# cyrillefavreau/Sol-R

Measured on AMD Instinct MI355X. Metric: Mrays/s @1920x1080, 3-bounce Cornell, higher is better.
Workload: dtype f32; 1 GPU; cornell 1920x1080, 3 bounces + shadow rays, 75 boxes / 29 primitives, one GPU, whole frame; rays_per_frame=6518779, closest_hit_walks_rank0=3506171, lane_nodes=206382796, lane_prim_tests=37557299, wave_nodes=3396811, wave_prim_tests=626627, wave_walks=106204, cost_ordered_launch_rank0=True, frames_in_flight=3, setup_frames_before_warmup=48, frames_delivered=9105, order_free_nodes=43, short_ray_lists=1, gather=none (one GPU), strips=equal rows, parallelism=tile1

## Files before the change

sol-r_amd/csrc/renderer.h:

```cpp
#ifndef SOLR_RENDERER_H
#define SOLR_RENDERER_H

#include <hip/hip_runtime.h>

#include "../../include/solr_hip.h"
#include "rt_device.h"

using namespace solrdev;

struct FrameArgs
{
    SceneInfo si;
    PostProcessingInfo ppi;
    float ox, oy, oz;
    float dx, dy, dz;
    float ax, ay, az, aw;
    Trig trig;
    float stepx, stepy;
    int firstRow;
    int nbRows;
    int tilesX;
    unsigned tileMagic;
    int tileShift;
    int fuseDefault;
// ... 46 lines not shown

struct PixelRecord
{
    float4 colorInfo;
    float4 sceneInfo;
};
static_assert(sizeof(PixelRecord) == sizeof(PostProcessingBuffer), "PixelRecord layout");


struct DepthHalo
{
    const float *above, *below;
    int nbAbove, nbBelow;
};

typedef void (*RendererFn)(const SceneArgs, const FrameArgs, PixelRecord *, int4 *, unsigned char *, unsigned long long *);
typedef void (*WalkBoundFn)(const SceneArgs, const char *, unsigned *, unsigned *);

namespace solrrows
{
struct Row
{
    int features;
    bool bothLoops;
};
constexpr Row ROWS[] = {
    {F_SPHERE | F_PLANE, true},
    {F_SPHERE | F_TRI, true},
    {F_SPHERE | F_CYL, true},
    {F_SPHERE | F_PLANE | F_TRI | F_CYL, false},
// ... 30 lines not shown
```

sol-r_amd/csrc/renderer_kernel.h:

```cpp
#ifndef SOLR_RENDERER_KERNEL_H
#define SOLR_RENDERER_KERNEL_H

#include "renderer.h"

using namespace solrdev;

template <int COUNT, int FEAT, bool VOLUME = false>
#ifndef SOLR_GENERIC_WAVES
#define SOLR_GENERIC_WAVES 0
#endif
#ifndef SOLR_WAVES_PER_EU
#define SOLR_WAVES_PER_EU 4
#endif
__global__ __launch_bounds__(WAVE, (SOLR_GENERIC_WAVES && (FEAT & F_TEX)) ? SOLR_GENERIC_WAVES : SOLR_WAVES_PER_EU) void k_standardRenderer(const SceneArgs SA, const FrameArgs F,
                                                           PixelRecord *__restrict__ pp,
                                                           int4 *__restrict__ ids, unsigned char *__restrict__ bitmap,
                                                           unsigned long long *__restrict__ counters)
{
    extern __shared__ float ldsStack[];
    const Scene S = makeScene(SA);
    const SceneInfo &si = F.si;
    const int lane = threadIdx.x;
    const unsigned entry = F.tileOrder ? F.tileOrder[blockIdx.x] : blockIdx.x;
    if (entry == ORDER_NOTHING)
        return;
    const int tile = (int)min(entry & ORDER_TILE_MASK, (unsigned)F.nbTiles - 1u);
    const int part = (int)((entry >> ORDER_PART_SHIFT) & 31u);
    unsigned long long clock0 = 0ull;
    if (F.tileClock || F.tileCost)
        clock0 = __builtin_amdgcn_s_memrealtime();
    const int ty = F.tileMagic ? (int)(__umulhi((unsigned)tile, F.tileMagic) >> F.tileShift) : tile;
    const int tx = tile - ty * F.tilesX;
    const int x = tx * TILE_W + (lane & (TILE_W - 1));
    const int yLocal = ty * TILE_H + (lane >> SOLR_TILE_W_LOG2);
    const int W = si.size.x;
    const bool mine = part == 0 || ((((lane & (TILE_W - 1)) >> (SOLR_TILE_W_LOG2 - SOLR_SPLIT_LOG2)) |
// ... 65 lines not shown
        rayD.y = rayD.y + F.stepy * (float)(yGlobal - (si.size.y / 2));
    }
    rayO = vectorRotation(rayO, rotationCenter, F.trig);
    rayD = vectorRotation(rayD, rotationCenter, F.trig);

    v3 color = V(0.f, 0.f, 0.f);
    if (!antialiasingActivated && (volume || si.pathTracingIteration >= NB_MAX_ITERATIONS))
    {
        const int k = si.pathTracingIteration % 4;
        rayD.x += (k == 0) ? 3.f : (k == 1) ? 5.f : (k == 2) ? -3.f : -5.f;
        rayD.y += (k == 0) ? 5.f : (k == 1) ? -3.f : (k == 2) ? -5.f : 3.f;
    }
    const bool anaglyph = (FEAT & F_FULL) && (si.cameraType == ctAnaglyph);
    const bool fishEye = (FEAT & F_FULL) && (si.cameraType == ctPanoramic);
    const bool vision = (FEAT & F_FULL) && (si.cameraType == ctVR);
    const bool plainStore = anaglyph || fishEye || vision;
    v3 leftEye = V(0.f, 0.f, 0.f);
    const int nbRays = antialiasingActivated ? 5 : (anaglyph ? 2 : 1);
#pragma unroll 1
    for (int I = 0; I < nbRays; ++I)
    {
        v3 rO = rayO;
        v3 rD = rayD;
        if (anaglyph)
        {
            const float stepx = F.stepx, stepy = F.stepy;
            rO = V((I == 0) ? F.ox - si.eyeSeparation : F.ox + si.eyeSeparation, F.oy, F.oz);
            rD = V(F.dx - stepx * (float)(x - (si.size.x / 2)), F.dy + stepy * (float)(yGlobal - (si.size.y / 2)), F.dz);
            rO = vectorRotation(rO, V(0.f, 0.f, 0.f), F.trig);
            rD = vectorRotation(rD, V(0.f, 0.f, 0.f), F.trig);
        }
        if (vision)
        {
            const float focus = fabsf(F.focusDepth - F.oz);
            const float eyeSeparation = si.eyeSeparation * (F.dz / focus);
            const int halfWidth = si.size.x / 2;
// ... 51 lines not shown
            }
            if (I >= 2)
            {
                rO.x += -3.f;
                rO.y += -5.f;
            }
            if (I >= 3)
            {
                rO.x += -5.f;
                rO.y += 3.f;
            }
        }
        v3 c;
        if constexpr (volume)
        {
            c = launchVolumeRendering<COUNT, FEAT>(S, active, gindex, rO, rD, si, F.ppi, id, cs, cnt);
            c = V(0.f + c.x, 0.f + c.y, 0.f + c.z);
        }
        else
            c = launchRayTracing<COUNT, FEAT>(S, active, gindex, rO, rD, si, dof, id, cs, cnt);
        if (anaglyph)
        {
            if (I == 0)
                leftEye = c;
            else
                color = V((leftEye.x * 0.299f + leftEye.y * 0.587f + leftEye.z * 0.114f) + 0.f, 0.f + c.y, 0.f + c.z);
        }
        else
            color = color + c;
    }

    SOLR_T(const unsigned long long tEpilogue0 = SOLR_NOW();)
    int tileAgain = tile, partAgain = part, laneAgain = (int)__builtin_amdgcn_mbcnt_hi(~0u, __builtin_amdgcn_mbcnt_lo(~0u, 0u));
    asm volatile("" : "+s"(tileAgain), "+s"(partAgain), "+v"(laneAgain));
    const int tyAgain = F.tileMagic ? (int)(__umulhi((unsigned)tileAgain, F.tileMagic) >> F.tileShift) : tileAgain;
    const int xAgain = (tileAgain - tyAgain * F.tilesX) * TILE_W + (laneAgain & (TILE_W - 1));
    const int yAgain = tyAgain * TILE_H + (laneAgain >> SOLR_TILE_W_LOG2);
    const int index = ((xAgain < si.size.x) && (yAgain < F.nbRows)) ? yAgain * si.size.x + xAgain : 0;
    const int gindexAgain = (F.firstRow + yAgain) * si.size.x + xAgain;

    if ((!plainStore || vision) && si.advancedIllumination == aiRandomIllumination)
    {
        int rindex = (gindexAgain + si.timestamp) % MAX_BITMAP_SIZE;
        float rv = rnd(S, rindex);
        color.x += si.backgroundColor.x * rv * 5.f;
        color.y += si.backgroundColor.y * rv * 5.f;
        color.z += si.backgroundColor.z * rv * 5.f;
    }
    if (antialiasingActivated)
    {
        color.x /= 5.f;
        color.y /= 5.f;
        color.z /= 5.f;
    }

    if (active)
    {
        float4 ppColor = make_float4(0.f, 0.f, 0.f, 0.f);
        float4 ppScene = make_float4(0.f, 0.f, 0.f, 0.f);
        if (si.pathTracingIteration > 0)
        {
            ppColor = pp[index].colorInfo;
            ppScene = pp[index].sceneInfo;
        }
        if (si.pathTracingIteration == 0)
            ppColor.w = dof;
        if (plainStore)
        {
            if (si.pathTracingIteration <= NB_MAX_ITERATIONS)
            {
                ppColor.x = color.x;
                ppColor.y = color.y;
                ppColor.z = color.z;
            }
            else
            {
                ppColor.x += color.x;
                ppColor.y += color.y;
                ppColor.z += color.z;
            }
        }
        else if (si.pathTracingIteration <= NB_MAX_ITERATIONS)
        {
            ppColor.x = color.x;
            ppColor.y = color.y;
            ppColor.z = color.z;
            ppScene.x = color.x;
            ppScene.y = color.y;
            ppScene.z = color.z;
        }
        else
        {
            ppScene.x = (id.z > 0) ? fmaxf(ppScene.x, color.x) : color.x;
            ppScene.y = (id.z > 0) ? fmaxf(ppScene.y, color.y) : color.y;
            ppScene.z = (id.z > 0) ? fmaxf(ppScene.z, color.z) : color.z;
            ppColor.x += ppScene.x;
            ppColor.y += ppScene.y;
            ppColor.z += ppScene.z;
        }
        pp[index].colorInfo = ppColor;
        pp[index].sceneInfo = ppScene;
        if ((FEAT & F_STREAM) && (F.fuseDefault & 4))
        {
            typedef int FourInts __attribute__((ext_vector_type(4)));
            const FourInts four = {id.x, id.y, id.z, id.w};
            asm volatile("global_store_dwordx4 %0, %1, off sc1" ::"v"(ids + index), "v"(four) : "memory");
        }
        else
            ids[index] = id;

        if (F.fuseDefault)
        {
            v3 c = V(ppColor.x, ppColor.y, ppColor.z);
            if (si.pathTracingIteration > NB_MAX_ITERATIONS)
            {
                float d = (float)(si.pathTracingIteration - NB_MAX_ITERATIONS + 1);
                c.x /= d;
                c.y /= d;
                c.z /= d;
            }
            if ((FEAT & F_STREAM) && (F.fuseDefault & 2))
                makeColor<true>(si, c, bitmap, index);
            else
                makeColor(si, c, bitmap, index);
        }
    }
    if ((FEAT & F_STREAM) && (F.fuseDefault & 2))
    {
        asm volatile("s_waitcnt vmcnt(0)" ::: "memory");
        const unsigned units = partAgain ? 1u : (unsigned)SPLIT_PARTS;
        unsigned before = 0u;
        if (laneAgain == 0)
            before = __hip_atomic_fetch_add(F.rowDone + 64 * tyAgain, units, __ATOMIC_RELAXED, __HIP_MEMORY_SCOPE_AGENT);
        before = (unsigned)__builtin_amdgcn_readfirstlane((int)before);
        if (before + units == F.streamSerial * (unsigned)(F.tilesX * SPLIT_PARTS) && laneAgain == 0)
        {
            const StreamPlan *plan = F.streamPlan;
            int band = 0;
            while (band + 1 < plan->bands && tyAgain >= plan->firstRow[band + 1])
                ++band;
            const int rows = plan->firstRow[band + 1] - plan->firstRow[band];
            const unsigned rowsBefore = __hip_atomic_fetch_add(plan->bandDone + 64 * band, 1u, __ATOMIC_RELAXED, __HIP_MEMORY_SCOPE_AGENT);
            if (rowsBefore + 1u == F.streamSerial * (unsigned)rows)
                __hip_atomic_store(plan->hostWord + band, F.streamSerial, __ATOMIC_RELAXED, __HIP_MEMORY_SCOPE_SYSTEM);
        }
    }

    if (F.tileClock && laneAgain == 0)
    {
        F.tileClock[2 * tileAgain] = clock0;
        F.tileClock[2 * tileAgain + 1] = __builtin_amdgcn_s_memrealtime();
    }
    if (F.tileCost && laneAgain == 0)
    {
        const unsigned cost = (unsigned)(__builtin_amdgcn_s_memrealtime() - clock0);
        F.tileCost[tileAgain] = partAgain ? (unsigned)(SOLR_SPLIT_LOG2 + 1) * cost : cost;
    }
#ifdef SOLR_TIMING
    if (COUNT == 0 && laneAgain == 0 && counters)
    {
        unsigned long long *slot = counters + 16 + 16ull * blockIdx.x;
        slot[0] += SOLR_NOW() - tKernel0;
        slot[8] += cnt.tShade;
        slot[9] += cnt.tTrace;
        slot[10] += SOLR_NOW() - tEpilogue0;
        slot[1] += cnt.tClosest;
        slot[2] += cnt.tShadow;
        slot[3] += cnt.tNode;
        slot[4] += cnt.tLeaf;
        slot[5] += (unsigned long long)cnt.nAdvance;
        slot[6] += (unsigned long long)cnt.nLeaf;
        slot[7] += 1ull;
        slot[11] += cnt.tClosestPrimary;
        slot[12] += cnt.tAgain;
        slot[13] += ((unsigned long long)cnt.nAgain << 32) | cnt.nAgainLanes;
        slot[14] += ((unsigned long long)cnt.nAdvanceFirst << 32) | cnt.nAdvanceAgain;
        slot[15] += (unsigned long long)cnt.nChecked;
    }
#endif
    if (COUNT == 2 && lane == 0)
        ((int4 *)cnt.record)[0] = make_int4((int)cnt.ordinal, 0, 0, 0);
    if (COUNT == 1)
    {
        unsigned int vals[4] = {cnt.closest, cnt.shadow, cnt.boxes, cnt.prims};
#pragma unroll
        for (int k = 0; k < 4; ++k)
        {
            unsigned int v = vals[k];
            for (int off = 32; off > 0; off >>= 1)
                v += __shfl_xor(v, off, 64);
            if (lane == 0)
                atomicAdd(&counters[k], (unsigned long long)v);
        }
        if (lane == 0)
        {
            atomicAdd(&counters[4], (unsigned long long)cnt.wNodes);
            atomicAdd(&counters[5], (unsigned long long)cnt.wPrims);
            atomicAdd(&counters[6], (unsigned long long)cnt.wClosest);
            atomicAdd(&counters[7], (unsigned long long)cnt.wShadow);
        }
    }
}

template <int FEAT>
__global__ __launch_bounds__(WAVE, SOLR_WAVES_PER_EU) void k_walkBound(const SceneArgs SA, const char *__restrict__ records,
                                                                       unsigned *__restrict__ visits, unsigned *__restrict__ skipped)
{
    extern __shared__ float ldsStack[];
    const Scene S = makeScene(SA);
    const int lane = threadIdx.x;
    const char *slot = records + (size_t)blockIdx.x * SOLR_WALK_SLOT_BYTES;
    const int4 *head = (const int4 *)slot;
    const float4 *rays = (const float4 *)(slot + 16 * (SOLR_WALK_SLOTS + 1));
    const int recorded = __builtin_amdgcn_readfirstlane(head[0].x);
// ... 64 lines not shown
```

sol-r_amd/csrc/rt_device.h:

```cpp
#pragma once

#include <hip/hip_runtime.h>
#include "pow_table.h"

#include "../../include/solr_types.h"
#include "scene_layout.h"

namespace solrdev
{
#define SOLR_DEV __device__ __forceinline__

struct v3
{
    float x, y, z;
};

SOLR_DEV v3 V(float x, float y, float z)
{
    v3 r;
    r.x = x;
    r.y = y;
    r.z = z;
    return r;
}
// ... 434 lines not shown


enum Feature
{
    F_SPHERE = 1,
    F_PROC = 2,
    F_CYL = 4,
    F_ELL = 8,
    F_TRI = 16,
    F_PLANE = 32,
    F_TEX = 64,
    F_FULL = 128,
    F_ALL = 255,
    F_DEEP = 256,
    F_STACK = 512,
    F_STREAM = 1024
};
#define SOLR_LDS_STACK_SLOTS 3

struct Hit
{
    v3 intersection;
    v3 normal;
    v3 areas;
    float shadowIntensity;
};

SOLR_DEV bool ellipsoidIntersection(const SceneInfo &si, v3 p0, v3 size, const WalkRay &ray, Hit &h)
{
    h.shadowIntensity = 1.f;
    v3 O_C = ray.o - p0;
    v3 dir = ray.dn;
// ... 816 lines not shown
}

SOLR_DEV bool longRay(v3 d)
{
    const float dd = dot(d, d);
    return dd >= 4.f && dd <= 1.0e24f;
}

SOLR_DEV bool tightRay(const WalkRay &r, const SceneInfo &si)
{
    return longRay(r.d) && r.d.x != 0.f && r.d.y != 0.f && r.d.z != 0.f && fabsf(r.o.x) <= si.viewDistance &&
           fabsf(r.o.y) <= si.viewDistance && fabsf(r.o.z) <= si.viewDistance;
}

template <int COUNT, int FEAT>
SOLR_DEV bool closestHitWalk(const Scene &S, const SceneInfo &si, bool active, v3 origin, v3 target, int iteration,
                             int currentMaterialId, int &closestPrimitive, v3 &closestIntersection,
                             v3 &closestNormal, v3 &closestAreas, v3 &colorBox, Counters &cnt)
{
    bool intersections = false;
    if (ballot(active) == 0ull)
        return false;
    SOLR_T(const unsigned long long tw0 = SOLR_NOW();)
    float minDistance = (iteration < 2) ? si.viewDistance : si.viewDistance / (iteration + 1);
    const WalkRay r = makeWalkRay(origin, target - origin);
    if (active)
        countAdd<COUNT>(cnt.closest, 1);
    countAdd<COUNT>(cnt.wClosest, 1);

    const bool fastBoxes = S.orderedBoxes && (ballot(active && !finiteRay(r)) == 0ull);
    const bool showBoxes = (FEAT & F_FULL) && si.renderBoxes != 0;
    const bool tidy = COUNT != 1 && fastBoxes && S.nested && !showBoxes;
    const bool freeOrder =
        tidy && S.nbBoxesFree > 0 && ballot(active && !longRay(r.d)) == 0ull;
    constexpr bool thinLeaves = (FEAT & F_PLANE) != 0;
    const bool tight = thinLeaves && tidy && S.tightLists && ballot(active && !tightRay(r, si)) == 0ull;
    const float ddShort = dot(r.d, r.d);
// ... 346 lines not shown
            break;
        SOLR_T(++cnt.nChecked;)
        const bool again = lanesNow && (intersections ? !(second > minDistance * rivalScale + slack) : bandHit);
        if (ballot(again) == 0ull)
            break;
        SOLR_T(++cnt.nAgain; cnt.nAgainLanes += (unsigned)__builtin_popcountll(ballot(again));)
        lanesNow = again;
        minDistance = again ? initialDistance : minDistance;
        intersections = again ? false : intersections;
    }
    SOLR_T(cnt.tClosest += SOLR_NOW() - tw0; if (iteration == 0) cnt.tClosestPrimary += SOLR_NOW() - tw0;)
    return intersections;
}

template <int COUNT, int FEAT>
SOLR_DEV float shadowWalk(const Scene &S, const SceneInfo &si, bool active, v3 lampCenter, v3 origin, int lightId,
                          int iteration, v3 &color, int objectId, Counters &cnt)
{
    float result = 0.f;
    color = V(0.f, 0.f, 0.f);
    if (ballot(active) == 0ull)
        return 0.f;
    SOLR_T(const unsigned long long tw0 = SOLR_NOW();)
    WalkRay r = makeWalkRay(origin, lampCenter - origin);
    r.o = origin + r.dn * si.rayEpsilon;
    const float minDistance = (iteration < 2) ? si.viewDistance : si.viewDistance / (iteration + 1);
    const float lengthOL = length(r.d);
    if (active)
        countAdd<COUNT>(cnt.shadow, 1);
    countAdd<COUNT>(cnt.wShadow, 1);

    const bool fastBoxes = S.orderedBoxes && (ballot(active && !finiteRay(r)) == 0ull);
    const bool tidy = COUNT != 1 && fastBoxes && S.nested;
    const bool freeOrder = tidy && S.nbBoxesFree > 0 && (S.opaqueShadows & SHADOWS_OPAQUE) &&
                           ballot(active && !(longRay(r.d) && minDistance >= 2.f)) == 0ull;
    const bool lampCut = tidy && !freeOrder && (S.opaqueShadows & SHADOWS_LAMP_CUTOFF);
    Scene W = S;
// ... 278 lines not shown
        }
    }
    else if (textured)
    {
        const float2 vt0 = make_float2(primRow(S, pi, ROW_N0).w, primRow(S, pi, ROW_N1).w);
        const float4 T = primRow(S, pi, ROW_UV);
        const float2 vt1 = make_float2(primRow(S, pi, ROW_N2).w, T.x);
        const float2 vt2 = make_float2(T.y, T.z);
        c = triangleUVMapping(si, vt0, vt1, vt2, mh.attributes.y, mh.color, loadMaterialCold(S, materialId), S.textures,
                              areas, o);
    }
    return c;
}

template <int COUNT, int FEAT>
SOLR_DEV v3 primitiveShader(const Scene &S, bool active, int index, const SceneInfo &si, v3 origin, v3 &normal,
                            int objectId, v3 intersection, v3 areas, v3 &closestColor, int iteration,
                            float &shadowIntensity, v3 &totalBlinn, float4 &attributes, Counters &cnt)
{
    SOLR_T(const unsigned long long tShade0 = SOLR_NOW();)
    const int pi = active ? objectId : 0;
    const int type = asint(primRow(S, pi, ROW_P0_TYPE).w) & PRIM_TYPE_MASK;
    const int materialId = asint(primRow(S, pi, ROW_SIZE_MAT).w);
    const int primIndex = asint(primRow(S, pi, ROW_P1_INDEX).w);
    const MaterialHot mh = loadMaterialHot(S, materialId);
    v3 lampsColor = V(0.f, 0.f, 0.f);
    v3 intersectionColor = V(0.f, 0.f, 0.f);
    float4 specular = make_float4(mh.specular.x, mh.specular.y, mh.specular.z, 0.f);
    float ambientOcclusion = 0.f;
    bool shade = active;

    if (active)
    {
        shadowIntensity = 0.f;
        v3 bumpNormal = V(0.f, 0.f, 0.f);
// ... 3 lines not shown
        normal = normal + bumpNormal;
        normal = normalize(normal);
        if (mh.attributes.z == 1)
            shade = false;
    }
    const bool wire = active && !shade;

    if (si.graphicsLevel > glNoShading)
    {
        if (shade)
        {
            closestColor.x *= mh.innerIllumination.x;
            closestColor.y *= mh.innerIllumination.x;
            closestColor.z *= mh.innerIllumination.x;
        }
        for (int cpt = 0; cpt < S.nbLights; ++cpt)
        {
            const int cptLamp =
                (si.pathTracingIteration >= NB_MAX_ITERATIONS) ? (si.pathTracingIteration % S.nbLights) : 0;
            const LightPlane li = loadLight(S, cptLamp);
            const int lightPrimitiveId = asint(li.location.w);
            const int lightMaterialId = li.materialId;
            const MaterialHot m = loadMaterialHot(S, lightMaterialId < 0 ? 0 : lightMaterialId);
            const bool lit = shade && (lightPrimitiveId != primIndex);

            v3 center = V4(li.location);
            const int t = (index + si.timestamp) % (MAX_BITMAP_SIZE - 3);
            if (si.pathTracingIteration >= NB_MAX_ITERATIONS)
            {
                float a = m.innerIllumination.y * 10.f * si.pathTracingIteration / si.maxPathTracingIterations;
                center.x += rnd(S, t) * a;
                center.y += rnd(S, t + 1) * a;
// ... 1 lines not shown
            }
            v3 lightRay = center - intersection;
            const float lightRayLength = length(lightRay);
            const bool inRange = lit && (lightRayLength < m.innerIllumination.z);
            v3 shadowColor = V(0.f, 0.f, 0.f);
            float lambert = 0.f;
            if (inRange)
            {
                lightRay = normalize(lightRay);
                lambert = mh.innerIllumination.x + dot(normal, lightRay);
            }
            const bool wantShadow = inRange && lambert > 0.f && si.graphicsLevel > 3 && iteration < 4 &&
                                    mh.innerIllumination.x == 0.f;
            {
                v3 sc;
                float s = shadowWalk<COUNT, FEAT>(S, si, wantShadow, center, intersection, lightPrimitiveId, iteration, sc,
                                            objectId, cnt);
                if (wantShadow)
                {
                    shadowIntensity = s;
                    shadowColor = sc;
                }
            }
            if (inRange)
            {
                float photonEnergy = sqrt_ieee(lightRayLength / m.innerIllumination.z);
                photonEnergy = (photonEnergy > 1.f) ? 1.f : photonEnergy;
                photonEnergy = (photonEnergy < 0.f) ? 0.f : photonEnergy;
                lambert *= (lambert < 0.f) ? -mh.transparency : 1.f;
                if (lightMaterialId != MATERIAL_NONE)
                    lambert *= m.innerIllumination.x;
                else
                    lambert *= li.color.w;
                if (mh.innerIllumination.w != 0.f)
                    lambert *= (1.f + rnd(S, t) * mh.innerIllumination.w * 100.f);
                lambert *= (1.f - shadowIntensity);
                lambert += si.backgroundColor.w;
                lambert *= (1.f - photonEnergy);
                lampsColor.x += lambert * li.color.x - shadowColor.x;
                lampsColor.y += lambert * li.color.y - shadowColor.y;
// ... 169 lines not shown
struct V3Ref
{
    float &x, &y, &z;
    SOLR_DEV V3Ref(const ColorStack &cs, int field) : x(cs.coldf(field)), y(cs.coldf(field + 1)), z(cs.coldf(field + 2)) {}
    SOLR_DEV operator v3() const { return V(x, y, z); }
    SOLR_DEV const V3Ref &operator=(const v3 &v) const
    {
        x = v.x;
        y = v.y;
        z = v.z;
        return *this;
    }
};

template <int COUNT, int FEAT>
SOLR_DEV v3 launchRayTracing(const Scene &S, bool active, int index, v3 rayO, v3 rayD, const SceneInfo &si,
                             float &depthOfField, int4 &primitiveXYId, const ColorStack &cs, Counters &cnt)
{
    SOLR_T(const unsigned long long tTrace0 = SOLR_NOW();)
    v3 intersectionColor = V(0.f, 0.f, 0.f);
    v3 closestIntersection = V(0.f, 0.f, 0.f);
    v3 normal = V(0.f, 0.f, 0.f);
    int closestPrimitive = -1;
    bool carryon = true;
    const V3Ref roO(cs, C_ROO), roD(cs, C_ROD);
    roO = rayO;
    roD = rayD;
    float &initialRefraction = cs.coldf(C_REFRACTION);
    initialRefraction = 1.f;
    int iteration = 0;
    int &lastIteration = cs.coldi(C_LASTIT);
    lastIteration = 0;
    int &idX = cs.coldi(C_ID_X), &idZ = cs.coldi(C_ID_Z), &idW = cs.coldi(C_ID_W);
    idX = -1;
// ... 42 lines not shown
    v3 ptO = V(0.f, 0.f, 0.f), ptD = V(0.f, 0.f, 0.f);
    float pathTracingRatio = 0.f;
    v3 pathTracingColor = V(0.f, 0.f, 0.f);
    bool useGlobalIllumination = false;
    bool test = true;

    v3 rBlinn = V(0.f, 0.f, 0.f);
    bool running = active;
    int phase = 0;

    while (true)
    {
        bool want;
        v3 tO, tD;
        int tIter, tMat;
        if (phase == 0)
        {
            running = running && (iteration < currentMaxIteration) && (rayLength < si.viewDistance) && carryon;
            if (ballot(running) == 0ull)
            {
                phase = 1;
                continue;
            }
            want = running;
            tO = roO;
            tD = roD;
            tIter = iteration;
            tMat = currentMaterialId;
        }
        else if (phase == 1)
// ... 2 lines not shown
            tO = rrO;
            tD = rrD;
            tIter = reflectedRays;
            tMat = currentMaterialId;
        }
        else
        {
            want = active && useGlobalIllumination && si.advancedIllumination == aiFull;
            tO = ptO;
            tD = ptD;
            tIter = 30;
            tMat = MATERIAL_NONE;
        }

        v3 areas = V(0.f, 0.f, 0.f);
        const bool hit = closestHitWalk<COUNT, FEAT>(S, si, want, tO, tD, tIter, tMat, closestPrimitive,
                                               closestIntersection, normal, areas, colorBox, cnt);
        const bool hitLane = want && hit;

        const int cp = hitLane ? closestPrimitive : 0;
        const int cpMaterial = asint(primRow(S, cp, ROW_SIZE_MAT).w);
        const MaterialHot cm = loadMaterialHot(S, cpMaterial < 0 ? 0 : cpMaterial);
        float4 attributes = make_float4(0.f, 0.f, 0.f, 0.f);
        bool shadeLane = hitLane;
        int shadeIteration = tIter;

        if (phase == 0)
        {
            if (running)
                carryon = hit;
            attributes = make_float4(cm.reflection, cm.transparency, cm.refraction, cm.opacity);
            if (hitLane)
            {
                currentMaterialId = cpMaterial;
                if (iteration == 0)
                {
                    cs.set(0, V(0.f, 0.f, 0.f));
                    cs.at(0, 3) = 1.f;
                    latestIntersection = closestIntersection;
                    dofCold = length(closestIntersection - tO);
                    if (giEnabled && cm.innerIllumination.x == 0.f)
                    {
                        int t = (index + si.pathTracingIteration * 100 + si.timestamp) % (MAX_BITMAP_SIZE - 3);
// ... 30 lines not shown
                        cs.at(0, 2) = cm.color.z * cm.innerIllumination.x * pathTracingRatio;
                        test = false;
                    }
                    else
                    {
                        cs.at(0, 0) = cm.color.x * pathTracingRatio;
                        cs.at(0, 1) = cm.color.y * pathTracingRatio;
                        cs.at(0, 2) = cm.color.z * pathTracingRatio;
                    }
                }
                if (test)
                {
                    pathTracingRatio *= STANDARD_LUNINANCE_STRENGTH;
                    if (cm.innerIllumination.x == 0.f)
                    {
                        cs.at(0, 0) -= si.shadowIntensity;
                        cs.at(0, 1) -= si.shadowIntensity;
                        cs.at(0, 2) -= si.shadowIntensity;
                    }
                    else
                        shadeLane = true;
                }
            }
            shadeIteration = lastIteration;
        }

        const v3 shaded = primitiveShader<COUNT, FEAT>(S, shadeLane, index, si, tO, normal, closestPrimitive,
                                                 closestIntersection, areas, closestColor, shadeIteration,
                                                 shadowIntensity, rBlinn, attributes, cnt);

        if (phase == 0)
        {
            if (hitLane)
            {
                v3 colorIt = shaded;
                float contribution;
                v3 reflectedTarget = V(0.f, 0.f, 0.f);
                idZ = (int)((float)idZ + cm.innerIllumination.x * 256);

                float segmentLength = length(closestIntersection - latestIntersection);
                latestIntersection = closestIntersection;

                float transparency = attributes.y;
                float a = 0.f;
                if (attributes.y != 0.f)
                {
                    float refraction = attributes.z;
// ... 84 lines not shown
        else if (phase == 1)
        {
            if (hitLane)
            {
                cs.template add<SP>(reflectedRays, V(shaded.x * reflectedRatio, shaded.y * reflectedRatio, shaded.z * reflectedRatio));
                idW = (int)(shadowIntensity * 255);
            }
            if (!giPass)
                break;
            phase = 2;
        }
        else
        {
            if (shadeLane)
                pathTracingColor = shaded;
            if (active && !hitLane && si.skyboxMaterialId != MATERIAL_NONE)
            {
                pathTracingColor = skyboxMapping<FEAT>(S, si, ptO, ptD);
                pathTracingRatio *= SKYBOX_LUNINANCE_STRENGTH;
            }
            if (active && test)
            {
                cs.at(0, 0) += pathTracingColor.x * pathTracingRatio;
                cs.at(0, 1) += pathTracingColor.y * pathTracingRatio;
                cs.at(0, 2) += pathTracingColor.z * pathTracingRatio;
            }
            break;
        }
    }

// ... 13 lines not shown
                const float4 cell = bs.template take<SP>(i);
                v3 ci = V(cell.x, cell.y, cell.z);
                float k = cell.w;
                next.x = ci.x * (1.f - k) + next.x * k;
                next.y = ci.y * (1.f - k) + next.y * k;
                next.z = ci.z * (1.f - k) + next.z * k;
            }
            intersectionColor = next;
            intersectionColor.x += recursiveBlinn.x;
            intersectionColor.y += recursiveBlinn.y;
            intersectionColor.z += recursiveBlinn.z;
        }
        else
            intersectionColor = cs.get(0);

        float D1 = si.viewDistance * 0.95f;
        const float dofNow = dofCold;
        if (si.atmosphericEffect == aeFog && dofNow > D1)
        {
            float D2 = si.viewDistance * 0.05f;
            float a = dofNow - D1;
            float b = 1.f - (a / D2);
            intersectionColor.x = intersectionColor.x * b + si.backgroundColor.x * (1.f - b);
            intersectionColor.y = intersectionColor.y * b + si.backgroundColor.y * (1.f - b);
            intersectionColor.z = intersectionColor.z * b + si.backgroundColor.z * (1.f - b);
        }
        intersectionColor.x -= colorBox.x;
        intersectionColor.y -= colorBox.y;
        intersectionColor.z -= colorBox.z;
    }
// ... 163 lines not shown
```

Baseline: 27680 Mrays/s.

## Read scene and frame args from kernarg segment to cut live registers

The renderer kernel now reads SceneArgs and FrameArgs through the kernarg segment pointer instead of copying them into locals. An opaque zero-offset helper (again<F_ARGS>) makes the compiler reload fields at each use rather than keep them live across the trace, shade and epilogue phases. The aim is lower SGPR/VGPR pressure and less spilling in the large kernel, at the cost of extra scalar loads. Triangle and textured variants keep their old behaviour.

```diff
diff --git a/sol-r_amd/csrc/renderer.h b/sol-r_amd/csrc/renderer.h
--- a/sol-r_amd/csrc/renderer.h
+++ b/sol-r_amd/csrc/renderer.h
@@ -84,6 +84,26 @@
     int nbAbove, nbBelow;
 };
 
+struct RendererArgs
+{
+    SceneArgs SA;
+    FrameArgs F;
+    PixelRecord *pp;
+    int4 *ids;
+    unsigned char *bitmap;
+    unsigned long long *counters;
+    __device__ __forceinline__ const Scene &scene() const { return *(const Scene *)&SA; }
+};
+static_assert(sizeof(Scene) == sizeof(SceneArgs) && alignof(Scene) == alignof(SceneArgs), "Scene is SceneArgs, retyped");
+static_assert(offsetof(Scene, offBoxes) == offsetof(SceneArgs, offBoxes) && offsetof(Scene, nbRandoms) == offsetof(SceneArgs, nbRandoms) &&
+                  offsetof(Scene, offLeaf) == offsetof(SceneArgs, offLeaf) && offsetof(Scene, sortedLists) == offsetof(SceneArgs, sortedLists),
+              "Scene is SceneArgs, retyped");
+static_assert(offsetof(RendererArgs, SA) == 0 && sizeof(RendererArgs) <= 512, "the kernel-argument segment of k_standardRenderer");
+__device__ __forceinline__ const RendererArgs &rendererArgs()
+{
+    return *(const RendererArgs *)(const SOLR_CONST_AS char *)__builtin_amdgcn_kernarg_segment_ptr();
+}
+
 typedef void (*RendererFn)(const SceneArgs, const FrameArgs, PixelRecord *, int4 *, unsigned char *, unsigned long long *);
 typedef void (*WalkBoundFn)(const SceneArgs, const char *, unsigned *, unsigned *);
 
diff --git a/sol-r_amd/csrc/renderer_kernel.h b/sol-r_amd/csrc/renderer_kernel.h
--- a/sol-r_amd/csrc/renderer_kernel.h
+++ b/sol-r_amd/csrc/renderer_kernel.h
@@ -12,14 +12,21 @@
 #ifndef SOLR_WAVES_PER_EU
 #define SOLR_WAVES_PER_EU 4
 #endif
-__global__ __launch_bounds__(WAVE, (SOLR_GENERIC_WAVES && (FEAT & F_TEX)) ? SOLR_GENERIC_WAVES : SOLR_WAVES_PER_EU) void k_standardRenderer(const SceneArgs SA, const FrameArgs F,
-                                                           PixelRecord *__restrict__ pp,
-                                                           int4 *__restrict__ ids, unsigned char *__restrict__ bitmap,
-                                                           unsigned long long *__restrict__ counters)
+__global__ __launch_bounds__(WAVE, (SOLR_GENERIC_WAVES && (FEAT & F_TEX)) ? SOLR_GENERIC_WAVES : SOLR_WAVES_PER_EU) void k_standardRenderer(const SceneArgs, const FrameArgs,
+                                                           PixelRecord *__restrict__,
+                                                           int4 *__restrict__, unsigned char *__restrict__,
+                                                           unsigned long long *__restrict__)
 {
     extern __shared__ float ldsStack[];
-    const Scene S = makeScene(SA);
+    constexpr int ARGS = FEAT | F_ARGS;
+    constexpr int TRACE = (FEAT & (F_TRI | F_TEX)) ? FEAT : ARGS;
+    const RendererArgs &A = rendererArgs();
+    const FrameArgs &F = A.F;
+    const Scene &S = A.scene();
     const SceneInfo &si = F.si;
+    PixelRecord *__restrict__ const pp = A.pp;
+    int4 *__restrict__ const ids = A.ids;
+    unsigned long long *__restrict__ const counters = A.counters;
     const int lane = threadIdx.x;
     const unsigned entry = F.tileOrder ? F.tileOrder[blockIdx.x] : blockIdx.x;
     if (entry == ORDER_NOTHING)
@@ -115,12 +122,13 @@
     const bool anaglyph = (FEAT & F_FULL) && (si.cameraType == ctAnaglyph);
     const bool fishEye = (FEAT & F_FULL) && (si.cameraType == ctPanoramic);
     const bool vision = (FEAT & F_FULL) && (si.cameraType == ctVR);
-    const bool plainStore = anaglyph || fishEye || vision;
     v3 leftEye = V(0.f, 0.f, 0.f);
     const int nbRays = antialiasingActivated ? 5 : (anaglyph ? 2 : 1);
 #pragma unroll 1
     for (int I = 0; I < nbRays; ++I)
     {
+        const FrameArgs &F = again<(FEAT & F_FULL) ? ARGS : 0>(A.F);
+        const SceneInfo &si = F.si;
         v3 rO = rayO;
         v3 rD = rayD;
         if (anaglyph)
@@ -202,11 +210,11 @@
         v3 c;
         if constexpr (volume)
         {
-            c = launchVolumeRendering<COUNT, FEAT>(S, active, gindex, rO, rD, si, F.ppi, id, cs, cnt);
+            c = launchVolumeRendering<COUNT, TRACE>(S, active, gindex, rO, rD, si, F.ppi, id, cs, cnt);
             c = V(0.f + c.x, 0.f + c.y, 0.f + c.z);
         }
         else
-            c = launchRayTracing<COUNT, FEAT>(S, active, gindex, rO, rD, si, dof, id, cs, cnt);
+            c = launchRayTracing<COUNT, TRACE>(S, active, gindex, rO, rD, si, dof, id, cs, cnt);
         if (anaglyph)
         {
             if (I == 0)
@@ -218,174 +226,187 @@
             color = color + c;
     }
 
-    SOLR_T(const unsigned long long tEpilogue0 = SOLR_NOW();)
-    int tileAgain = tile, partAgain = part, laneAgain = (int)__builtin_amdgcn_mbcnt_hi(~0u, __builtin_amdgcn_mbcnt_lo(~0u, 0u));
-    asm volatile("" : "+s"(tileAgain), "+s"(partAgain), "+v"(laneAgain));
-    const int tyAgain = F.tileMagic ? (int)(__umulhi((unsigned)tileAgain, F.tileMagic) >> F.tileShift) : tileAgain;
-    const int xAgain = (tileAgain - tyAgain * F.tilesX) * TILE_W + (laneAgain & (TILE_W - 1));
-    const int yAgain = tyAgain * TILE_H + (laneAgain >> SOLR_TILE_W_LOG2);
-    const int index = ((xAgain < si.size.x) && (yAgain < F.nbRows)) ? yAgain * si.size.x + xAgain : 0;
-    const int gindexAgain = (F.firstRow + yAgain) * si.size.x + xAgain;
-
-    if ((!plainStore || vision) && si.advancedIllumination == aiRandomIllumination)
-    {
-        int rindex = (gindexAgain + si.timestamp) % MAX_BITMAP_SIZE;
-        float rv = rnd(S, rindex);
-        color.x += si.backgroundColor.x * rv * 5.f;
-        color.y += si.backgroundColor.y * rv * 5.f;
-        color.z += si.backgroundColor.z * rv * 5.f;
-    }
-    if (antialiasingActivated)
-    {
-        color.x /= 5.f;
-        color.y /= 5.f;
-        color.z /= 5.f;
-    }
-
-    if (active)
-    {
-        float4 ppColor = make_float4(0.f, 0.f, 0.f, 0.f);
-        float4 ppScene = make_float4(0.f, 0.f, 0.f, 0.f);
-        if (si.pathTracingIteration > 0)
-        {
-            ppColor = pp[index].colorInfo;
-            ppScene = pp[index].sceneInfo;
-        }
-        if (si.pathTracingIteration == 0)
-            ppColor.w = dof;
-        if (plainStore)
-        {
-            if (si.pathTracingIteration <= NB_MAX_ITERATIONS)
+    {
+        SOLR_T(const unsigned long long tEpilogue0 = SOLR_NOW();)
+        int tileAgain = tile, partAgain = part, laneAgain = (int)__builtin_amdgcn_mbcnt_hi(~0u, __builtin_amdgcn_mbcnt_lo(~0u, 0u));
+        asm volatile("" : "+s"(tileAgain), "+s"(partAgain), "+v"(laneAgain));
+        const RendererArgs &E = again<ARGS>(A);
+        const FrameArgs &F = E.F;
+        const Scene &S = E.scene();
+        const SceneInfo &si = F.si;
+        PixelRecord *__restrict__ const pp = E.pp;
+        int4 *__restrict__ const ids = E.ids;
+        unsigned char *__restrict__ const bitmap = E.bitmap;
+        unsigned long long *__restrict__ const counters = E.counters;
+        const bool antialiasingActivated = (FEAT & F_FULL) && (si.cameraType == ctAntialiazed);
+        const bool vision = (FEAT & F_FULL) && (si.cameraType == ctVR);
+        const bool plainStore = vision || ((FEAT & F_FULL) && (si.cameraType == ctAnaglyph || si.cameraType == ctPanoramic));
+        const int tyAgain = F.tileMagic ? (int)(__umulhi((unsigned)tileAgain, F.tileMagic) >> F.tileShift) : tileAgain;
+        const int xAgain = (tileAgain - tyAgain * F.tilesX) * TILE_W + (laneAgain & (TILE_W - 1));
+        const int yAgain = tyAgain * TILE_H + (laneAgain >> SOLR_TILE_W_LOG2);
+        const int index = ((xAgain < si.size.x) && (yAgain < F.nbRows)) ? yAgain * si.size.x + xAgain : 0;
+        const int gindexAgain = (F.firstRow + yAgain) * si.size.x + xAgain;
+
+        if ((!plainStore || vision) && si.advancedIllumination == aiRandomIllumination)
+        {
+            int rindex = (gindexAgain + si.timestamp) % MAX_BITMAP_SIZE;
+            float rv = rnd(S, rindex);
+            color.x += si.backgroundColor.x * rv * 5.f;
+            color.y += si.backgroundColor.y * rv * 5.f;
+            color.z += si.backgroundColor.z * rv * 5.f;
+        }
+        if (antialiasingActivated)
+        {
+            color.x /= 5.f;
+            color.y /= 5.f;
+            color.z /= 5.f;
+        }
+
+        if (active)
+        {
+            float4 ppColor = make_float4(0.f, 0.f, 0.f, 0.f);
+            float4 ppScene = make_float4(0.f, 0.f, 0.f, 0.f);
+            if (si.pathTracingIteration > 0)
+            {
+                ppColor = pp[index].colorInfo;
+                ppScene = pp[index].sceneInfo;
+            }
+            if (si.pathTracingIteration == 0)
+                ppColor.w = dof;
+            if (plainStore)
+            {
+                if (si.pathTracingIteration <= NB_MAX_ITERATIONS)
+                {
+                    ppColor.x = color.x;
+                    ppColor.y = color.y;
+                    ppColor.z = color.z;
+                }
+                else
+                {
+                    ppColor.x += color.x;
+                    ppColor.y += color.y;
+                    ppColor.z += color.z;
+                }
+            }
+            else if (si.pathTracingIteration <= NB_MAX_ITERATIONS)
             {
                 ppColor.x = color.x;
                 ppColor.y = color.y;
                 ppColor.z = color.z;
+                ppScene.x = color.x;
+                ppScene.y = color.y;
+                ppScene.z = color.z;
             }
             else
             {
-                ppColor.x += color.x;
-                ppColor.y += color.y;
-                ppColor.z += color.z;
-            }
-        }
-        else if (si.pathTracingIteration <= NB_MAX_ITERATIONS)
-        {
-            ppColor.x = color.x;
-            ppColor.y = color.y;
-            ppColor.z = color.z;
-            ppScene.x = color.x;
-            ppScene.y = color.y;
-            ppScene.z = color.z;
-        }
-        else
-        {
-            ppScene.x = (id.z > 0) ? fmaxf(ppScene.x, color.x) : color.x;
-            ppScene.y = (id.z > 0) ? fmaxf(ppScene.y, color.y) : color.y;
-            ppScene.z = (id.z > 0) ? fmaxf(ppScene.z, color.z) : color.z;
-            ppColor.x += ppScene.x;
-            ppColor.y += ppScene.y;
-            ppColor.z += ppScene.z;
-        }
-        pp[index].colorInfo = ppColor;
-        pp[index].sceneInfo = ppScene;
-        if ((FEAT & F_STREAM) && (F.fuseDefault & 4))
-        {
-            typedef int FourInts __attribute__((ext_vector_type(4)));
-            const FourInts four = {id.x, id.y, id.z, id.w};
-            asm volatile("global_store_dwordx4 %0, %1, off sc1" ::"v"(ids + index), "v"(four) : "memory");
-        }
-        else
-            ids[index] = id;
-
-        if (F.fuseDefault)
-        {
-            v3 c = V(ppColor.x, ppColor.y, ppColor.z);
-            if (si.pathTracingIteration > NB_MAX_ITERATIONS)
-            {
-                float d = (float)(si.pathTracingIteration - NB_MAX_ITERATIONS + 1);
-                c.x /= d;
-                c.y /= d;
-                c.z /= d;
-            }
-            if ((FEAT & F_STREAM) && (F.fuseDefault & 2))
-                makeColor<true>(si, c, bitmap, index);
+                ppScene.x = (id.z > 0) ? fmaxf(ppScene.x, color.x) : color.x;
+                ppScene.y = (id.z > 0) ? fmaxf(ppScene.y, color.y) : color.y;
+                ppScene.z = (id.z > 0) ? fmaxf(ppScene.z, color.z) : color.z;
+                ppColor.x += ppScene.x;
+                ppColor.y += ppScene.y;
+                ppColor.z += ppScene.z;
+            }
+            pp[index].colorInfo = ppColor;
+            pp[index].sceneInfo = ppScene;
+            if ((FEAT & F_STREAM) && (F.fuseDefault & 4))
+            {
+                typedef int FourInts __attribute__((ext_vector_type(4)));
+                const FourInts four = {id.x, id.y, id.z, id.w};
+                asm volatile("global_store_dwordx4 %0, %1, off sc1" ::"v"(ids + index), "v"(four) : "memory");
+            }
             else
-                makeColor(si, c, bitmap, index);
-        }
-    }
-    if ((FEAT & F_STREAM) && (F.fuseDefault & 2))
-    {
-        asm volatile("s_waitcnt vmcnt(0)" ::: "memory");
-        const unsigned units = partAgain ? 1u : (unsigned)SPLIT_PARTS;
-        unsigned before = 0u;
-        if (laneAgain == 0)
-            before = __hip_atomic_fetch_add(F.rowDone + 64 * tyAgain, units, __ATOMIC_RELAXED, __HIP_MEMORY_SCOPE_AGENT);
-        before = (unsigned)__builtin_amdgcn_readfirstlane((int)before);
-        if (before + units == F.streamSerial * (unsigned)(F.tilesX * SPLIT_PARTS) && laneAgain == 0)
-        {
-            const StreamPlan *plan = F.streamPlan;
-            int band = 0;
-            while (band + 1 < plan->bands && tyAgain >= plan->firstRow[band + 1])
-                ++band;
-            const int rows = plan->firstRow[band + 1] - plan->firstRow[band];
-            const unsigned rowsBefore = __hip_atomic_fetch_add(plan->bandDone + 64 * band, 1u, __ATOMIC_RELAXED, __HIP_MEMORY_SCOPE_AGENT);
-            if (rowsBefore + 1u == F.streamSerial * (unsigned)rows)
-                __hip_atomic_store(plan->hostWord + band, F.streamSerial, __ATOMIC_RELAXED, __HIP_MEMORY_SCOPE_SYSTEM);
-        }
-    }
-
-    if (F.tileClock && laneAgain == 0)
-    {
-        F.tileClock[2 * tileAgain] = clock0;
-        F.tileClock[2 * tileAgain + 1] = __builtin_amdgcn_s_memrealtime();
-    }
-    if (F.tileCost && laneAgain == 0)
-    {
-        const unsigned cost = (unsigned)(__builtin_amdgcn_s_memrealtime() - clock0);
-        F.tileCost[tileAgain] = partAgain ? (unsigned)(SOLR_SPLIT_LOG2 + 1) * cost : cost;
-    }
+                ids[index] = id;
+
+            if (F.fuseDefault)
+            {
+                v3 c = V(ppColor.x, ppColor.y, ppColor.z);
+                if (si.pathTracingIteration > NB_MAX_ITERATIONS)
+                {
+                    float d = (float)(si.pathTracingIteration - NB_MAX_ITERATIONS + 1);
+                    c.x /= d;
+                    c.y /= d;
+                    c.z /= d;
+                }
+                if ((FEAT & F_STREAM) && (F.fuseDefault & 2))
+                    makeColor<true>(si, c, bitmap, index);
+                else
+                    makeColor(si, c, bitmap, index);
+            }
+        }
+        if ((FEAT & F_STREAM) && (F.fuseDefault & 2))
+        {
+            asm volatile("s_waitcnt vmcnt(0)" ::: "memory");
+            const unsigned units = partAgain ? 1u : (unsigned)SPLIT_PARTS;
+            unsigned before = 0u;
+            if (laneAgain == 0)
+                before = __hip_atomic_fetch_add(F.rowDone + 64 * tyAgain, units, __ATOMIC_RELAXED, __HIP_MEMORY_SCOPE_AGENT);
+            before = (unsigned)__builtin_amdgcn_readfirstlane((int)before);
+            if (before + units == F.streamSerial * (unsigned)(F.tilesX * SPLIT_PARTS) && laneAgain == 0)
+            {
+                const StreamPlan *plan = F.streamPlan;
+                int band = 0;
+                while (band + 1 < plan->bands && tyAgain >= plan->firstRow[band + 1])
+                    ++band;
+                const int rows = plan->firstRow[band + 1] - plan->firstRow[band];
+                const unsigned rowsBefore = __hip_atomic_fetch_add(plan->bandDone + 64 * band, 1u, __ATOMIC_RELAXED, __HIP_MEMORY_SCOPE_AGENT);
+                if (rowsBefore + 1u == F.streamSerial * (unsigned)rows)
+                    __hip_atomic_store(plan->hostWord + band, F.streamSerial, __ATOMIC_RELAXED, __HIP_MEMORY_SCOPE_SYSTEM);
+            }
+        }
+
+        if (F.tileClock && laneAgain == 0)
+        {
+            F.tileClock[2 * tileAgain] = clock0;
+            F.tileClock[2 * tileAgain + 1] = __builtin_amdgcn_s_memrealtime();
+        }
+        if (F.tileCost && laneAgain == 0)
+        {
+            const unsigned cost = (unsigned)(__builtin_amdgcn_s_memrealtime() - clock0);
+            F.tileCost[tileAgain] = partAgain ? (unsigned)(SOLR_SPLIT_LOG2 + 1) * cost : cost;
+        }
 #ifdef SOLR_TIMING
-    if (COUNT == 0 && laneAgain == 0 && counters)
-    {
-        unsigned long long *slot = counters + 16 + 16ull * blockIdx.x;
-        slot[0] += SOLR_NOW() - tKernel0;
-        slot[8] += cnt.tShade;
-        slot[9] += cnt.tTrace;
-        slot[10] += SOLR_NOW() - tEpilogue0;
-        slot[1] += cnt.tClosest;
-        slot[2] += cnt.tShadow;
-        slot[3] += cnt.tNode;
-        slot[4] += cnt.tLeaf;
-        slot[5] += (unsigned long long)cnt.nAdvance;
-        slot[6] += (unsigned long long)cnt.nLeaf;
-        slot[7] += 1ull;
-        slot[11] += cnt.tClosestPrimary;
-        slot[12] += cnt.tAgain;
-        slot[13] += ((unsigned long long)cnt.nAgain << 32) | cnt.nAgainLanes;
-        slot[14] += ((unsigned long long)cnt.nAdvanceFirst << 32) | cnt.nAdvanceAgain;
-        slot[15] += (unsigned long long)cnt.nChecked;
-    }
-#endif
-    if (COUNT == 2 && lane == 0)
-        ((int4 *)cnt.record)[0] = make_int4((int)cnt.ordinal, 0, 0, 0);
-    if (COUNT == 1)
-    {
-        unsigned int vals[4] = {cnt.closest, cnt.shadow, cnt.boxes, cnt.prims};
+        if (COUNT == 0 && laneAgain == 0 && counters)
+        {
+            unsigned long long *slot = counters + 16 + 16ull * blockIdx.x;
+            slot[0] += SOLR_NOW() - tKernel0;
+            slot[8] += cnt.tShade;
+            slot[9] += cnt.tTrace;
+            slot[10] += SOLR_NOW() - tEpilogue0;
+            slot[1] += cnt.tClosest;
+            slot[2] += cnt.tShadow;
+            slot[3] += cnt.tNode;
+            slot[4] += cnt.tLeaf;
+            slot[5] += (unsigned long long)cnt.nAdvance;
+            slot[6] += (unsigned long long)cnt.nLeaf;
+            slot[7] += 1ull;
+            slot[11] += cnt.tClosestPrimary;
+            slot[12] += cnt.tAgain;
+            slot[13] += ((unsigned long long)cnt.nAgain << 32) | cnt.nAgainLanes;
+            slot[14] += ((unsigned long long)cnt.nAdvanceFirst << 32) | cnt.nAdvanceAgain;
+            slot[15] += (unsigned long long)cnt.nChecked;
+        }
+#endif
+        if (COUNT == 2 && lane == 0)
+            ((int4 *)cnt.record)[0] = make_int4((int)cnt.ordinal, 0, 0, 0);
+        if (COUNT == 1)
+        {
+            unsigned int vals[4] = {cnt.closest, cnt.shadow, cnt.boxes, cnt.prims};
 #pragma unroll
-        for (int k = 0; k < 4; ++k)
-        {
-            unsigned int v = vals[k];
-            for (int off = 32; off > 0; off >>= 1)
-                v += __shfl_xor(v, off, 64);
+            for (int k = 0; k < 4; ++k)
+            {
+                unsigned int v = vals[k];
+                for (int off = 32; off > 0; off >>= 1)
+                    v += __shfl_xor(v, off, 64);
+                if (lane == 0)
+                    atomicAdd(&counters[k], (unsigned long long)v);
+            }
             if (lane == 0)
-                atomicAdd(&counters[k], (unsigned long long)v);
-        }
-        if (lane == 0)
-        {
-            atomicAdd(&counters[4], (unsigned long long)cnt.wNodes);
-            atomicAdd(&counters[5], (unsigned long long)cnt.wPrims);
-            atomicAdd(&counters[6], (unsigned long long)cnt.wClosest);
-            atomicAdd(&counters[7], (unsigned long long)cnt.wShadow);
+            {
+                atomicAdd(&counters[4], (unsigned long long)cnt.wNodes);
+                atomicAdd(&counters[5], (unsigned long long)cnt.wPrims);
+                atomicAdd(&counters[6], (unsigned long long)cnt.wClosest);
+                atomicAdd(&counters[7], (unsigned long long)cnt.wShadow);
+            }
         }
     }
 }
diff --git a/sol-r_amd/csrc/rt_device.h b/sol-r_amd/csrc/rt_device.h
--- a/sol-r_amd/csrc/rt_device.h
+++ b/sol-r_amd/csrc/rt_device.h
@@ -472,8 +472,22 @@
     F_ALL = 255,
     F_DEEP = 256,
     F_STACK = 512,
-    F_STREAM = 1024
+    F_STREAM = 1024,
+    F_ARGS = 2048
 };
+
+template <int FEAT, class T>
+SOLR_DEV const T &again(const T &v)
+{
+    if constexpr ((FEAT & F_ARGS) != 0)
+    {
+        int zero = 0;
+        asm volatile("" : "+s"(zero));
+        return *(const T *)((const char *)&v + zero);
+    }
+    else
+        return v;
+}
 #define SOLR_LDS_STACK_SLOTS 3
 
 struct Hit
@@ -1320,13 +1334,15 @@
 }
 
 template <int COUNT, int FEAT>
-SOLR_DEV bool closestHitWalk(const Scene &S, const SceneInfo &si, bool active, v3 origin, v3 target, int iteration,
+SOLR_DEV bool closestHitWalk(const Scene &S_, const SceneInfo &si_, bool active, v3 origin, v3 target, int iteration,
                              int currentMaterialId, int &closestPrimitive, v3 &closestIntersection,
                              v3 &closestNormal, v3 &closestAreas, v3 &colorBox, Counters &cnt)
 {
     bool intersections = false;
     if (ballot(active) == 0ull)
         return false;
+    const Scene S = again<FEAT>(S_);
+    const SceneInfo si = again<FEAT>(si_);
     SOLR_T(const unsigned long long tw0 = SOLR_NOW();)
     float minDistance = (iteration < 2) ? si.viewDistance : si.viewDistance / (iteration + 1);
     const WalkRay r = makeWalkRay(origin, target - origin);
@@ -1703,13 +1719,15 @@
 }
 
 template <int COUNT, int FEAT>
-SOLR_DEV float shadowWalk(const Scene &S, const SceneInfo &si, bool active, v3 lampCenter, v3 origin, int lightId,
+SOLR_DEV float shadowWalk(const Scene &S_, const SceneInfo &si_, bool active, v3 lampCenter, v3 origin, int lightId,
                           int iteration, v3 &color, int objectId, Counters &cnt)
 {
     float result = 0.f;
     color = V(0.f, 0.f, 0.f);
     if (ballot(active) == 0ull)
         return 0.f;
+    const Scene S = again<FEAT>(S_);
+    const SceneInfo si = again<FEAT>(si_);
     SOLR_T(const unsigned long long tw0 = SOLR_NOW();)
     WalkRay r = makeWalkRay(origin, lampCenter - origin);
     r.o = origin + r.dn * si.rayEpsilon;
@@ -2018,11 +2036,13 @@
 }
 
 template <int COUNT, int FEAT>
-SOLR_DEV v3 primitiveShader(const Scene &S, bool active, int index, const SceneInfo &si, v3 origin, v3 &normal,
+SOLR_DEV v3 primitiveShader(const Scene &S_, bool active, int index, const SceneInfo &si_, v3 origin, v3 &normal,
                             int objectId, v3 intersection, v3 areas, v3 &closestColor, int iteration,
                             float &shadowIntensity, v3 &totalBlinn, float4 &attributes, Counters &cnt)
 {
     SOLR_T(const unsigned long long tShade0 = SOLR_NOW();)
+    const Scene S = again<FEAT>(S_);
+    const SceneInfo si = again<FEAT>(si_);
     const int pi = active ? objectId : 0;
     const int type = asint(primRow(S, pi, ROW_P0_TYPE).w) & PRIM_TYPE_MASK;
     const int materialId = asint(primRow(S, pi, ROW_SIZE_MAT).w);
@@ -2056,8 +2076,10 @@
             closestColor.y *= mh.innerIllumination.x;
             closestColor.z *= mh.innerIllumination.x;
         }
-        for (int cpt = 0; cpt < S.nbLights; ++cpt)
-        {
+        for (int cpt = 0; cpt < again<FEAT>(S_).nbLights; ++cpt)
+        {
+            const Scene S = again<FEAT>(S_);
+            const SceneInfo si = again<FEAT>(si_);
             const int cptLamp =
                 (si.pathTracingIteration >= NB_MAX_ITERATIONS) ? (si.pathTracingIteration % S.nbLights) : 0;
             const LightPlane li = loadLight(S, cptLamp);
@@ -2089,7 +2111,7 @@
                                     mh.innerIllumination.x == 0.f;
             {
                 v3 sc;
-                float s = shadowWalk<COUNT, FEAT>(S, si, wantShadow, center, intersection, lightPrimitiveId, iteration, sc,
+                float s = shadowWalk<COUNT, FEAT>(S_, si_, wantShadow, center, intersection, lightPrimitiveId, iteration, sc,
                                             objectId, cnt);
                 if (wantShadow)
                 {
@@ -2099,6 +2121,8 @@
             }
             if (inRange)
             {
+                const Scene S = again<FEAT>(S_);
+                const SceneInfo si = again<FEAT>(si_);
                 float photonEnergy = sqrt_ieee(lightRayLength / m.innerIllumination.z);
                 photonEnergy = (photonEnergy > 1.f) ? 1.f : photonEnergy;
                 photonEnergy = (photonEnergy < 0.f) ? 0.f : photonEnergy;
@@ -2298,10 +2322,11 @@
 };
 
 template <int COUNT, int FEAT>
-SOLR_DEV v3 launchRayTracing(const Scene &S, bool active, int index, v3 rayO, v3 rayD, const SceneInfo &si,
+SOLR_DEV v3 launchRayTracing(const Scene &S_, bool active, int index, v3 rayO, v3 rayD, const SceneInfo &si_,
                              float &depthOfField, int4 &primitiveXYId, const ColorStack &cs, Counters &cnt)
 {
     SOLR_T(const unsigned long long tTrace0 = SOLR_NOW();)
+    const SceneInfo si = again<FEAT>(si_);
     v3 intersectionColor = V(0.f, 0.f, 0.f);
     v3 closestIntersection = V(0.f, 0.f, 0.f);
     v3 normal = V(0.f, 0.f, 0.f);
@@ -2374,6 +2399,7 @@
         bool want;
         v3 tO, tD;
         int tIter, tMat;
+        const SceneInfo si = again<FEAT>(si_);
         if (phase == 0)
         {
             running = running && (iteration < currentMaxIteration) && (rayLength < si.viewDistance) && carryon;
@@ -2406,9 +2432,10 @@
         }
 
         v3 areas = V(0.f, 0.f, 0.f);
-        const bool hit = closestHitWalk<COUNT, FEAT>(S, si, want, tO, tD, tIter, tMat, closestPrimitive,
+        const bool hit = closestHitWalk<COUNT, FEAT>(S_, si_, want, tO, tD, tIter, tMat, closestPrimitive,
                                                closestIntersection, normal, areas, colorBox, cnt);
         const bool hitLane = want && hit;
+        const Scene S = again<FEAT>(S_);
 
         const int cp = hitLane ? closestPrimitive : 0;
         const int cpMaterial = asint(primRow(S, cp, ROW_SIZE_MAT).w);
@@ -2419,6 +2446,7 @@
 
         if (phase == 0)
         {
+            const SceneInfo si = again<FEAT>(si_);
             if (running)
                 carryon = hit;
             attributes = make_float4(cm.reflection, cm.transparency, cm.refraction, cm.opacity);
@@ -2479,6 +2507,7 @@
                     pathTracingRatio *= STANDARD_LUNINANCE_STRENGTH;
                     if (cm.innerIllumination.x == 0.f)
                     {
+                        const SceneInfo &si = again<FEAT>(si_);
                         cs.at(0, 0) -= si.shadowIntensity;
                         cs.at(0, 1) -= si.shadowIntensity;
                         cs.at(0, 2) -= si.shadowIntensity;
@@ -2490,12 +2519,14 @@
             shadeIteration = lastIteration;
         }
 
-        const v3 shaded = primitiveShader<COUNT, FEAT>(S, shadeLane, index, si, tO, normal, closestPrimitive,
+        const v3 shaded = primitiveShader<COUNT, FEAT>(S_, shadeLane, index, si_, tO, normal, closestPrimitive,
                                                  closestIntersection, areas, closestColor, shadeIteration,
                                                  shadowIntensity, rBlinn, attributes, cnt);
 
         if (phase == 0)
         {
+            const Scene S = again<FEAT>(S_);
+            const SceneInfo si = again<FEAT>(si_);
             if (hitLane)
             {
                 v3 colorIt = shaded;
@@ -2610,6 +2641,8 @@
         {
             if (shadeLane)
                 pathTracingColor = shaded;
+            const Scene &S = again<FEAT>(S_);
+            const SceneInfo &si = again<FEAT>(si_);
             if (active && !hitLane && si.skyboxMaterialId != MATERIAL_NONE)
             {
                 pathTracingColor = skyboxMapping<FEAT>(S, si, ptO, ptD);
@@ -2653,6 +2686,7 @@
         else
             intersectionColor = cs.get(0);
 
+        const SceneInfo si = again<FEAT>(si_);
         float D1 = si.viewDistance * 0.95f;
         const float dofNow = dofCold;
         if (si.atmosphericEffect == aeFog && dofNow > D1)
```

Result: faster. 28530 Mrays/s (median of 6 runs) (+3.1%).
